# om-ai-lab/OmChat

Measured on AMD Instinct MI355X. Metric: images/sec prefill + decode tokens/sec, OmChat-13B TP=1/8; p50 TTFT, higher is better.
Workload: dtype bf16

## Files before the change

omchat_amd/csrc/attention.hip:

```cpp
#include "kernels.h"

#include "attn_common.h"

namespace {

__device__ __forceinline__ float max3(float a, float b, float c) {
  float r;
  asm("v_max3_f32 %0, %1, %2, %3" : "=v"(r) : "v"(a), "v"(b), "v"(c));
  return r;
}
__device__ __forceinline__ float max2(float a, float b) {
  float r;
  asm("v_max_f32 %0, %1, %2" : "=v"(r) : "v"(a), "v"(b));
  return r;
}
__device__ __forceinline__ float max_xor32_raw(float v) {
  const auto r = __builtin_amdgcn_permlane32_swap(__float_as_uint(v), __float_as_uint(v), false, false);
  return max2(__uint_as_float(r[0]), __uint_as_float(r[1]));
}
__device__ __forceinline__ float max_xor16_raw(float v) {
  const auto r = __builtin_amdgcn_permlane16_swap(__float_as_uint(v), __float_as_uint(v), false, false);
  return max2(__uint_as_float(r[0]), __uint_as_float(r[1]));
}

// ... 228 lines not shown
  extern __shared__ __attribute__((aligned(256))) char smem_all[];

  const int tid = threadIdx.x % NT, lane = tid & 63;
  const int wave_all = __builtin_amdgcn_readfirstlane((int)threadIdx.x >> 6);
  const int kg = KG == 1 ? 0 : wave_all / (NW / KG);
  const int wave = KG == 1 ? wave_all : wave_all % (NW / KG);
  char* const smem = smem_all + kg * 2 * BUF;
  const int qc = lane & 31, hh = lane >> 5;

  const int n_rep = p.q_heads / p.kv_heads;
  const int nb = GQA ? p.nsplit : 1;
  const int per_rank = GQA ? p.kv_heads * nb : 1;
  const int xs = GQA ? p.tpw : 0;
  const int nqb = GQA ? (int)gridDim.x / per_rank - xs : (p.tpw == -1 ? (p.nsplit & 0xffff) : (int)gridDim.x);
  int h_lo = 0, h_hi = GQA ? n_rep : 1, bx, rest;
  if (GQA && (int)blockIdx.x < 2 * xs * per_rank) {
    const int pair = (int)blockIdx.x >> 1;
    bx = pair / per_rank; rest = pair % per_rank;
    if (blockIdx.x & 1) h_lo = (n_rep + 1) / 2; else h_hi = (n_rep + 1) / 2;
  } else if (GQA) {
    const int j = (int)blockIdx.x - 2 * xs * per_rank;
    bx = xs + j / per_rank; rest = j % per_rank;
  } else {
    bx = (int)blockIdx.x; rest = 0;
  }
  int mha_head = (int)blockIdx.y, mha_b = (int)blockIdx.z;
  if (!GQA && p.tpw == -1) {
    const int nq = p.nsplit & 0xffff, nbat = p.nsplit >> 16, grp = (int)blockIdx.x / (8 * nq), r = (int)blockIdx.x % (8 * nq);
    const int pair = grp * 8 + (r & 7);
    bx = r >> 3;
    if (pair >= p.q_heads * nbat) return;
    mha_head = pair % p.q_heads; mha_b = pair / p.q_heads;
  }
  const int qb = p.causal ? nqb - 1 - bx : bx;
  const int b = GQA ? rest / p.kv_heads : mha_b;
  constexpr int QW = GQA ? 32 : (NW / KG) * 32;
  const int kvh = GQA ? rest % p.kv_heads : mha_head / n_rep;
  const int hq = GQA ? kvh * n_rep + wave : mha_head;
  const int q0b = qb * QW;
  const int q0 = q0b + (GQA ? 0 : wave * 32);
  const int kv_len = p.kv_len ? p.kv_len[b] : p.Skv;
  const int kv_start = p.kv_start ? p.kv_start[b] : 0;
  const bool peel = !GQA && KG == 1 && D == 128 && p.peel_last && !p.causal && kv_start == 0 && kv_len > KV_TILE && (kv_len & (KV_TILE - 1)) == 1;
  int kmax = peel ? kv_len - 1 : kv_len;
  if (p.causal) { const int lim = q0b + QW + p.q_pos0; kmax = lim < kmax ? lim : kmax; }
  const int t_end = (kmax + KV_TILE - 1) / KV_TILE;
  const int t_begin = kv_start / KV_TILE;

  const T* Kg = (const T*)p.K + b * p.k_sb + kvh * p.k_sh;
  const T* Vg = (const T*)p.V + b * p.v_sb + kvh * p.v_sh;
  const bool wave_active = (GQA ? (wave >= h_lo && wave < h_hi) : true) && q0 < p.Sq;

  frag_t qf[KS];
  const int qrow = q0 + qc;
  {
    const int rr = qrow < p.Sq ? qrow : p.Sq - 1;
    const T* qp = (const T*)p.Q + b * p.q_sb + (wave_active ? hq : 0) * p.q_sh + (int64_t)rr * p.q_sr;
#pragma unroll
    for (int s = 0; s < KS; ++s) qf[s] = ld8<T>(qp + s * 16 + hh * 8);
  }
  [[maybe_unused]] float qn_ss = 0.f;
  [[maybe_unused]] frag_t qn_wv[(!GQA && D == 128) ? KS : 1];
  if constexpr (!GQA && D == 128) {
    if (p.qn_sumsq) {
      const int rr = qrow < p.Sq ? qrow : p.Sq - 1;
      qn_ss = p.qn_sumsq[((size_t)b * p.Sq + rr) * p.qn_stride];
      const T* wq = (const T*)p.qn_w + (size_t)hq * D;
#pragma unroll
      for (int s = 0; s < KS; ++s) qn_wv[s] = ld8<T>(wq + s * 16 + hh * 8);
// ... 1178 lines not shown
int g_attn_v2 = 1;
void attn_set_v2(int v) { g_attn_v2 = v; }

namespace {
template <typename T>
__global__ __launch_bounds__(128) void attn_uniform_rows_kernel(AttnP p) {
  const int h = blockIdx.x, b = blockIdx.y, d = threadIdx.x;
  const int start = p.kv_start[b];
  if (start <= 0) return;
  const int kvh = h / (p.q_heads / p.kv_heads);
  const T* V = (const T*)p.V + b * p.v_sb + kvh * p.v_sh + d;
  const float w = rnd<T>(1.0f / (float)p.Skv);
  float acc = 0.f;
  for (int j = 0; j < p.Skv; ++j) acc += w * tof(V[(int64_t)j * p.v_sr]);
  const T o = fromf<T>(acc);
  T* O = (T*)p.O + b * p.o_sb + h * p.o_sh + d;
  for (int i = 0; i < start && i < p.Sq; ++i) O[(int64_t)i * p.o_sr] = o;
}
}

int launch_attn_uniform_rows(int dtype, const AttnArgs& a, hipStream_t s) {
  OM_CHECK(a.kv_start && (a.head_dim == 0 || a.head_dim == 128), "uniform rows: left-padded batch (kv_start), head dim 128");
  AttnP p{a.Q, a.K, a.V, a.O, a.q_sb, a.q_sh, a.q_sr, a.k_sb, a.k_sh, a.k_sr, a.v_sb, a.v_sh, a.v_sr, a.o_sb, a.o_sh, a.o_sr,
          a.kv_len, a.kv_start, a.q_heads, a.kv_heads, a.Sq, a.Skv, a.causal, a.q_pos0, 0, a.scale * 1.4426950408889634f, nullptr,
          nullptr, nullptr, nullptr, nullptr, 0, nullptr, nullptr, 0, nullptr, nullptr, 0, 0, 0, nullptr, 0};
  const dim3 grid(a.q_heads, a.batch);
  if (dtype == OMCHAT_F16) hipLaunchKernelGGL(attn_uniform_rows_kernel<f16>, grid, dim3(128), 0, s, p);
  else if (dtype == OMCHAT_BF16) hipLaunchKernelGGL(attn_uniform_rows_kernel<bf16>, grid, dim3(128), 0, s, p);
  else { omchat_set_error("launch_attn_uniform_rows: bad dtype"); return 1; }
  OM_LAUNCH_CHECK();
  return 0;
}

int launch_attn_prefill(int dtype, const AttnArgs& a, hipStream_t s) {
  OM_CHECK(a.q_heads % a.kv_heads == 0, "q_heads must be a multiple of kv_heads");
  OM_CHECK(a.Sq > 0 && a.Skv > 0 && a.batch > 0, "empty attention");
  OM_CHECK(a.q_sr % 8 == 0 && a.k_sr % 8 == 0 && a.v_sr % 8 == 0 && a.o_sr % 4 == 0, "row strides must keep 16-B alignment");
  AttnP p{a.Q, a.K, a.V, a.O, a.q_sb, a.q_sh, a.q_sr, a.k_sb, a.k_sh, a.k_sr, a.v_sb, a.v_sh, a.v_sr, a.o_sb, a.o_sh, a.o_sr,
          a.kv_len, a.kv_start, a.q_heads, a.kv_heads, a.Sq, a.Skv, a.causal, a.q_pos0, 0, a.scale * 1.4426950408889634f, nullptr,
          nullptr, nullptr, nullptr, nullptr, 0, nullptr, nullptr, 0, nullptr, nullptr, 0, 0, 0, nullptr, 0};
  dim3 grid(cdiv(a.Sq, 128), a.q_heads, a.batch);
  p.peel_last = g_attn_peel;
  const int hd = a.head_dim ? a.head_dim : 128;
  OM_CHECK(hd == 128 || hd == 64, "head_dim must be 128 or 64");
  if (a.qn_sumsq) {
    OM_CHECK(a.q_heads == a.kv_heads && hd == 128 && g_attn_v2 && !a.causal && a.qn_w && a.qn_stride >= 1 && a.qn_dim > 0,
             "q norm on load: MHA at head dim 128 on the second-generation kernel");
    p.qn_sumsq = a.qn_sumsq; p.qn_stride = a.qn_stride; p.qn_dim = a.qn_dim; p.qn_w = a.qn_w; p.qn_eps = a.qn_eps; p.qn_scale = a.qn_scale;
  }
  dim3 grid_x = grid;
  if (g_attn_mha_xcd && !a.causal && grid.x < 65536 && a.batch < 32768) { p.tpw = -1; p.nsplit = (int)grid.x | (a.batch << 16); grid_x = dim3(cdiv(a.q_heads * a.batch, 8) * 8 * grid.x, 1, 1); }
  constexpr int LDS128 = 2 * 2 * KV_TILE * 256;
  auto use_kg2 = [&](int per_cu1, int per_cu2) {
    if (!OMCHAT_EXPERIMENTS || g_attn_kg != 2) return false;
    if (a.causal || a.kv_start || a.q_heads != a.kv_heads) return false;
    if (g_attn_kg) return g_attn_kg == 2;
    const long wgs = (long)grid.x * a.q_heads * a.batch, G = device_cus();
    const long r1 = (wgs + G * per_cu1 - 1) / (G * per_cu1), r2 = (wgs + G * per_cu2 - 1) / (G * per_cu2);
    return 2 * r1 > r2 + (r1 > 4 ? 1 : 0) && cdiv(a.Skv, KV_TILE) >= 4;
  };
  if (hd == 64 && g_attn_v2 && a.q_heads == a.kv_heads) {
    const bool kg2 = use_kg2(4, 2); (void)kg2;
    constexpr int LDS64 = 2 * 2 * KV_TILE * 128;
#if OMCHAT_EXPERIMENTS
    if (kg2 && dtype == OMCHAT_F16) OM_LAUNCH_ATTN2((attn2_kernel<f16, 8, false, 64, 2>), grid_x, 512, 2 * LDS64);
    else if (kg2 && dtype == OMCHAT_BF16) OM_LAUNCH_ATTN2((attn2_kernel<bf16, 8, false, 64, 2>), grid_x, 512, 2 * LDS64);
    else
#endif
    if (dtype == OMCHAT_F16) OM_LAUNCH_ATTN2((attn2_kernel<f16, 4, false, 64>), grid_x, 256, LDS64);
    else if (dtype == OMCHAT_BF16) OM_LAUNCH_ATTN2((attn2_kernel<bf16, 4, false, 64>), grid_x, 256, LDS64);
    else { omchat_set_error("launch_attn_prefill: bad dtype"); return 1; }
    OM_LAUNCH_CHECK();
    return 0;
  }
  if (hd == 64) {
    if (dtype == OMCHAT_F16) hipLaunchKernelGGL((attn_kernel<f16, 4, 2, 64>), grid, dim3(256), 0, s, p);
    else if (dtype == OMCHAT_BF16) hipLaunchKernelGGL((attn_kernel<bf16, 4, 2, 64>), grid, dim3(256), 0, s, p);
    else { omchat_set_error("launch_attn_prefill: bad dtype"); return 1; }
    OM_LAUNCH_CHECK();
    return 0;
  }
  const int n_rep = a.q_heads / a.kv_heads;
  if (g_attn_v2 && n_rep == 1) {
    const bool kg2 = use_kg2(2, 1); (void)kg2;
#if OMCHAT_EXPERIMENTS
    if (kg2 && dtype == OMCHAT_F16) OM_LAUNCH_ATTN2((attn2_kernel<f16, 8, false, 128, 2>), grid_x, 512, 2 * LDS128);
    else if (kg2 && dtype == OMCHAT_BF16) OM_LAUNCH_ATTN2((attn2_kernel<bf16, 8, false, 128, 2>), grid_x, 512, 2 * LDS128);
    else
#endif
    if (dtype == OMCHAT_F16) OM_LAUNCH_ATTN2((attn2_kernel<f16, 4, false>), grid_x, 256, LDS128);
    else if (dtype == OMCHAT_BF16) OM_LAUNCH_ATTN2((attn2_kernel<bf16, 4, false>), grid_x, 256, LDS128);
    else { omchat_set_error("launch_attn_prefill: bad dtype"); return 1; }
    OM_LAUNCH_CHECK();
    return 0;
  }
  if (g_attn_v2 && n_rep <= 8) {
    const int nqb_ = cdiv(a.Sq, 32), per_rank = a.kv_heads * a.batch;
    int xs = 0;
    if (a.causal && n_rep >= 4 && !a.kv_start && (long)nqb_ * per_rank <= device_cus() && nqb_ >= 16)
      xs = g_attn_hsplit >= 0 ? std::min(g_attn_hsplit, nqb_ / 2) : nqb_ / 4;
    if (g_attn_hsplit > 0 && a.causal && n_rep >= 4 && !a.kv_start && nqb_ >= 16) xs = std::min(g_attn_hsplit, nqb_ / 2);
    const dim3 g2((nqb_ + xs) * per_rank, 1, 1);
    p.nsplit = a.batch; p.tpw = xs;
#define OM_A2(NW_)                                                                                                       \
  do {                                                                                                                   \
    if (dtype == OMCHAT_F16) OM_LAUNCH_ATTN2((attn2_kernel<f16, NW_, true>), g2, NW_ * 64, LDS128);                      \
    else if (dtype == OMCHAT_BF16) OM_LAUNCH_ATTN2((attn2_kernel<bf16, NW_, true>), g2, NW_ * 64, LDS128);               \
    else { omchat_set_error("launch_attn_prefill: bad dtype"); return 1; }                                               \
  } while (0)
    switch (n_rep) { case 2: OM_A2(2); break; case 3: OM_A2(3); break; case 4: OM_A2(4); break; case 5: OM_A2(5); break;
                     case 6: OM_A2(6); break; case 7: OM_A2(7); break; default: OM_A2(8); break; }
#undef OM_A2
    OM_LAUNCH_CHECK();
    return 0;
  }
  if (dtype == OMCHAT_F16) hipLaunchKernelGGL((attn_kernel<f16, 4, 2, 128>), grid, dim3(256), 0, s, p);
  else if (dtype == OMCHAT_BF16) hipLaunchKernelGGL((attn_kernel<bf16, 4, 2, 128>), grid, dim3(256), 0, s, p);
  else { omchat_set_error("launch_attn_prefill: bad dtype"); return 1; }
  OM_LAUNCH_CHECK();
  return 0;
}

size_t attn_decode_ws_bytes(int batch, int q_heads, int max_len) {
  return (size_t)batch * q_heads * cdiv(max_len, KV_TILE) * WS_STRIDE * sizeof(float);
}

static void kv8_plan(int batch, int kv_heads, int L, bool masked, int* tpw, int* nw) {
  *tpw = 1; *nw = 1;
  if (masked) return;
  const long waves1 = (long)cdiv(L, KV_TILE) * kv_heads * batch;
  if (g_attn_kv8_tpw > 0) { *tpw = g_attn_kv8_tpw & 7; *nw = (g_attn_kv8_tpw & 8) ? 4 : 1; }
  else {
    *tpw = waves1 >= 2L * device_cus() ? 3 : 1;
    const int n4 = cdiv(L, 12 * KV_TILE);
    if (*tpw == 3 && n4 <= 64 && (long)n4 * kv_heads * batch >= device_cus() / 2) *nw = 4;
  }
// ... 369 lines not shown
```

omchat_amd/csrc/attn_common.h:

```cpp
#pragma once
#include "kernels.h"

namespace {


struct AttnP {
  const void* Q; const void* K; const void* V; void* O;
  int64_t q_sb, q_sh, q_sr, k_sb, k_sh, k_sr, v_sb, v_sh, v_sr, o_sb, o_sh, o_sr;
  const int* kv_len;
  const int* kv_start;
  int q_heads, kv_heads, Sq, Skv, causal, q_pos0, nsplit;
  float c;
  float* ws;
  const float* rope;
  const int* pos;
  const void* k_new; const void* v_new; int64_t new_sb;
  void* k_cache_w; void* v_cache_w;
  int rope_max;
  const float* k_scale; const float* v_scale; int64_t scale_sb, scale_sh;
  int tpw;
  const unsigned char* key_mask; int64_t mask_sb;
  const float* qn_sumsq = nullptr; int qn_stride = 0, qn_dim = 0; const void* qn_w = nullptr; float qn_eps = 0.f, qn_scale = 1.f;
  int peel_last = 0;
#if OMCHAT_EXPERIMENTS
  unsigned long long* dbg;
#endif
};

template <typename T> __device__ __forceinline__ typename V8<T>::type widen8(u32x2 w);
template <> __device__ __forceinline__ bf16x8 widen8<bf16>(u32x2 w) {
  typedef bf16 v2 __attribute__((ext_vector_type(2)));
  const v2 a = __builtin_amdgcn_cvt_scalef32_pk_bf16_fp8(w.x, 1.0f, false), b = __builtin_amdgcn_cvt_scalef32_pk_bf16_fp8(w.x, 1.0f, true);
  const v2 c = __builtin_amdgcn_cvt_scalef32_pk_bf16_fp8(w.y, 1.0f, false), d = __builtin_amdgcn_cvt_scalef32_pk_bf16_fp8(w.y, 1.0f, true);
  return (bf16x8){a[0], a[1], b[0], b[1], c[0], c[1], d[0], d[1]};
}
template <> __device__ __forceinline__ f16x8 widen8<f16>(u32x2 w) {
  typedef f16 v2 __attribute__((ext_vector_type(2)));
  const v2 a = __builtin_amdgcn_cvt_scalef32_pk_f16_fp8(w.x, 1.0f, false), b = __builtin_amdgcn_cvt_scalef32_pk_f16_fp8(w.x, 1.0f, true);
  const v2 c = __builtin_amdgcn_cvt_scalef32_pk_f16_fp8(w.y, 1.0f, false), d = __builtin_amdgcn_cvt_scalef32_pk_f16_fp8(w.y, 1.0f, true);
  return (f16x8){a[0], a[1], b[0], b[1], c[0], c[1], d[0], d[1]};
}

template <typename T>
__device__ __forceinline__ typename V8<T>::type rope_chunk(typename V8<T>::type x, typename V8<T>::type o, const float* cs, bool second_half) {
#pragma clang fp contract(off)
  typename V8<T>::type r;
  const float sgn = second_half ? 1.f : -1.f;
#pragma unroll
  for (int j = 0; j < 8; ++j) {
    const float co = rnd<T>(cs[2 * j]), si = rnd<T>(cs[2 * j + 1]);
    r[j] = fromf<T>(rnd<T>(tof(x[j]) * co) + rnd<T>(sgn * tof(o[j]) * si));
  }
  return r;
}

constexpr int KV_TILE = 64;
// ... 227 lines not shown
```

omchat_amd/csrc/capi.hip:

```cpp
#include "kernels.h"
#include <stdlib.h>
#include "../../include/omchat_hip.h"
#include <math.h>
#include <vector>

#define S(x) ((hipStream_t)(x))
#if OMCHAT_EXPERIMENTS
int g_launch_any_order = 0;
#endif

extern "C" int omchat_op_gemm(int dtype, const void* A, int lda, const void* W, int ldw, void* C, int ldc, int M, int N, int K,
                              const void* bias, const void* ls, const void* resid, int ldr, int epi, int force_tile, void* stream) {
  GemmArgs g{A, lda, W, ldw, C, ldc, M, N, K, bias, ls, resid, ldr, epi, force_tile, nullptr, 0, -1};
  return launch_gemm(dtype, g, S(stream));
}

extern "C" int omchat_op_gemm_fused(int dtype, const void* A, int lda, const void* W, int ldw, void* C, int ldc, int M, int N, int K,
                                    const void* bias, const void* ls, const void* resid, int ldr, int epi, int force_tile, const float* row_scale,
                                    const float* rs_stats, int rs_ld, int rs_nslots, int rs_dim, float rs_eps,
                                    float* stats, int stats_ld, int* nslots, void* stream) {
  GemmArgs g{A, lda, W, ldw, C, ldc, M, N, K, bias, ls, resid, ldr, epi, force_tile, nullptr, 0, -1};
  g.row_scale = row_scale; g.stats = stats; g.stats_ld = stats_ld; g.stats_nslots = nslots;
  g.rs_stats = rs_stats; g.rs_ld = rs_ld; g.rs_nslots = rs_nslots; g.rs_dim = rs_dim; g.rs_eps = rs_eps;
  return launch_gemm(dtype, g, S(stream));
// ... 39 lines not shown
  if (key == 6) { model_set_pack_replica(value); return 0; }
  if (key == 8) { attn_set_v2(value); return 0; }
  if (key == 9) { model_set_fuse_peer_norm(value); return 0; }
  if (key == 10) { attn_set_tpw(value); return 0; }
  if (key == 11) { gemv_set_no_xs(value); return 0; }
  if (key == 12) { attn_set_klds(value); return 0; }
  if (key == 25) { attn_set_dma(value); return 0; }
  if (key == 26) { attn_set_dma_slots(value); return 0; }
  if (key == 27) { attn_set_dma_rot(value); return 0; }
  if (key == 28) { gemv_set_skew(value); return 0; }
  if (key == 29) { model_set_tp_f32(value); return 0; }
  if (key == 30) { attn_set_hsplit(value); return 0; }
  if (key == 33) { attn_set_mha_xcd(value); return 0; }
  if (key == 16) { gemv_set_norm_loop(value); return 0; }
  if (key == 17) { gemv_set_rows_balance(value); return 0; }
  if (key == 19) { attn_set_merge_mid_min(value); return 0; }
  if (key == 21) { attn_set_merge_dg(value); return 0; }
  if (key == 13) { gemm_set_persist(value); return 0; }
  if (key == 14) { model_set_norm_in_gemv(value); return 0; }
  if (key == 22) { model_set_fuse_attn_oproj(value); return 0; }
  if (key == 23) { model_set_decode_layer(value); return 0; }
  if (key == 24) { gemv_set_dyn(value); return 0; }
  if (key == 34) { gemv_set_shard_shapes(value); return 0; }
  if (key == 35) { model_set_shard_as_tp1(value); return 0; }
  if (key == 36) { attn_set_kg(value); return 0; }
  if (key == 37) { gemm_set_wide_store(value); return 0; }
  if (key == 43) { gemm_set_skip_dead(value); return 0; }
  if (key == 44) { model_set_vit_fused(value); return 0; }
  if (key == 45) { model_set_tp_sp(value); return 0; }
  if (key == 46) { attn_set_peel(value); return 0; }
  if (key == 47) { attn_set_kv8_tpw(value); return 0; }
  if (key == 48) { attn_set_kv8_fuse(value); return 0; }
  if (key == 49) { model_set_extend_attn(value); return 0; }
  if (key == 38) { gemv_set_gu_rr(value); return 0; }
  if (key == 39) { gemv_set_longk_direct(value); return 0; }
  if (key == 40) { norm_set_wave(value); return 0; }
#if OMCHAT_EXPERIMENTS
  if (key == 41) { g_launch_any_order = value; return 0; }
  if (key == 42) { model_set_ao_oproj(value); return 0; }
#endif
  omchat_set_error("omchat_op_set_tuning: unknown key");
  return 1;
}

extern "C" int omchat_allreduce_noop(void*, void*, size_t, int, void*) { return 0; }

extern "C" int omchat_gemm_tune_load(const char* path) { OM_CHECK(path, "null path"); return gemm_tune_load(path); }
extern "C" int omchat_gemm_tune_dump(const char* path) { OM_CHECK(path, "null path"); return gemm_tune_dump(path); }
extern "C" long omchat_gemm_tune_runs(void) { return gemm_tune_runs(); }

extern "C" size_t omchat_op_gemm_sk_ws(void) { return gemm_sk_ws_bytes(); }

extern "C" int omchat_op_gemm_sk(int dtype, const void* A, int lda, const void* W, int ldw, void* C, int ldc, int M, int N, int K,
                                 const void* bias, const void* ls, const void* resid, int ldr, int epi, int force_tile, void* ws,
                                 size_t ws_bytes, int stream_k, void* stream) {
  GemmArgs g{A, lda, W, ldw, C, ldc, M, N, K, bias, ls, resid, ldr, epi, force_tile, ws, ws_bytes, stream_k};
  return launch_gemm(dtype, g, S(stream));
}

extern "C" int omchat_op_gemv(int dtype, const void* X, int ldx, const void* W, int ldw, void* Y, int ldy, int b, int N, int K,
                              const void* bias, const void* resid, int ldr, int epi, int out_f32, void* stream) {
  GemvArgs g{X, ldx, W, ldw, Y, ldy, b, N, K, bias, resid, ldr, epi, out_f32};
  return launch_gemv(dtype, g, S(stream));
}

extern "C" int omchat_op_gemv_norm(int dtype, const void* X, const void* W, int ldw, void* Y, int N, int K, const void* norm_w, float eps,
// ... 383 lines not shown
```

omchat_amd/csrc/kernels.h:

```cpp
#pragma once
#ifndef OMCHAT_EXPERIMENTS
#define OMCHAT_EXPERIMENTS 0
#endif
#include "common.h"
#if OMCHAT_EXPERIMENTS
#include <hip/hip_ext.h>
extern int g_launch_any_order;
#undef hipLaunchKernelGGL
#define hipLaunchKernelGGL(kernelName, numBlocks, numThreads, memPerBlock, streamId, ...)                                                      \
  do {                                                                                                                                         \
    if (g_launch_any_order)                                                                                                                    \
      hipExtLaunchKernelGGL((kernelName), dim3(numBlocks), dim3(numThreads), (memPerBlock), (streamId), nullptr, nullptr, hipExtAnyOrderLaunch, \
                            __VA_ARGS__);                                                                                                      \
    else                                                                                                                                       \
      hipLaunchKernelGGLInternal((kernelName), numBlocks, numThreads, memPerBlock, streamId, __VA_ARGS__);                                     \
  } while (0)
#endif

enum {
  EPI_NONE = 0,
  EPI_GELU = 1,
  EPI_LS_RESID = 2,
  EPI_RESID = 3,
  EPI_SWIGLU = 4,
// ... 66 lines not shown
void model_set_pack_replica(int v);
void model_set_norm_in_gemv(int v);
void model_set_vit_fused(int v);
void model_set_tp_sp(int v);
int launch_fold_cols(int dtype, const void* W, const void* n, void* out, int rows, int cols, hipStream_t s);

int launch_layernorm(int dtype, const void* x, int ldx, const void* w, const void* b, void* y, int ldy, int rows, int H, float eps, hipStream_t stream);
int launch_rmsnorm(int dtype, const void* x, int ldx, const void* w, void* y, int ldy, int rows, int H, float eps, hipStream_t s, int pack_nb = 0);
int launch_rmsnorm_q8(int dtype, const void* x, int ldx, const void* w, void* y8, int ldy, float* scale, int rows, int H, float eps, hipStream_t s);
int launch_quant_rows_q8(int dtype, const void* x, int ldx, void* y8, int ldy, float* scale, int rows, int H, hipStream_t s);
int launch_resid_rmsnorm(int dtype, void* x, int ldx, const float* part, int ks, const void* w, void* xn, int ldn, int rows, int H, float eps,
                         hipStream_t s, int pack_nb = 0);
int launch_resid16_norm(int dtype, void* x, int ldx, const void* y, int ldy, const void* w, const void* b, void* xn, int ldn, int rows, int H, float eps,
                        hipStream_t s);
int launch_vit_qknorm(int dtype, void* qkv, int ld, const void* wq, const void* wk, int rows, int C, int C_total,
                      float eps, float q_scale, const float* sumsq_in, hipStream_t s, int only_k = 0);
int launch_vit_qk_sumsq(int dtype, const void* qkv, int ld, int rows, int C, float* sumsq_out, hipStream_t s);
int launch_vit_knorm_slots(int dtype, void* k, int ld, const void* wk, int rows, int C, int C_total, float eps, const float* stats, int stats_ld, int nslots,
                           float* sumsq_q, hipStream_t s);
struct AttnArgs {
  const void* Q; int64_t q_sb, q_sh, q_sr;
  const void* K; int64_t k_sb, k_sh, k_sr;
  const void* V; int64_t v_sb, v_sh, v_sr;
  void* O; int64_t o_sb, o_sh, o_sr;
  int batch, q_heads, kv_heads;
  int Sq, Skv;
  const int* kv_len;
  const int* kv_start;
  int causal;
  int q_pos0;
  float scale;
  int head_dim;
  const float* qn_sumsq = nullptr; int qn_stride = 0, qn_dim = 0; const void* qn_w = nullptr; float qn_eps = 0.f, qn_scale = 1.f;
};
int launch_attn_prefill(int dtype, const AttnArgs& a, hipStream_t s);
int launch_attn_uniform_rows(int dtype, const AttnArgs& a, hipStream_t s);
void attn_set_v2(int v);
void model_set_fuse_peer_norm(int v);
void attn_set_tpw(int v);
void attn_set_klds(int v);
void attn_set_dma(int v);
void attn_set_dma_slots(int v);
void attn_set_dma_rot(int v);
void attn_set_hsplit(int v);
void attn_set_mha_xcd(int v);
void attn_set_kg(int v);
void attn_set_peel(int v);
void attn_set_kv8_tpw(int v);
void attn_set_kv8_fuse(int v);
void model_set_extend_attn(int v);
bool attn_decode_kv8_fuses_rope(int batch, int kv_heads, int L, bool masked);
void attn_set_merge_mid_min(int v);
void attn_set_merge_dg(int v);
void gemv_set_norm_loop(int v);
void gemv_set_dyn(int v);
void gemv_set_skew(int v);
void gemv_set_rows_balance(int v);
void gemv_set_no_xs(int v);
void gemv_set_shard_shapes(int v);
void gemv_set_gu_rr(int v);
void gemv_set_longk_direct(int v);
void norm_set_wave(int v);
void model_set_ao_oproj(int v);
int gemv_get_shard_shapes();

struct AttnDecodeArgs {
  const void* Q; int64_t q_sb, q_sh;
  const void* K; int64_t k_sb, k_sh, k_sr;
  const void* V; int64_t v_sb, v_sh, v_sr;
  void* O; int64_t o_sb, o_sh;
  int batch, q_heads, kv_heads;
  int L;
  const int* kv_len;
  float scale;
  float* ws; size_t ws_bytes;
  const float* rope; int rope_max;
  const int* pos;
  const void* k_new; const void* v_new; int64_t new_sb;
  int o_pack_nb;
  const float* k_scale; const float* v_scale; int64_t scale_sb, scale_sh;
  void* k16_w = nullptr; void* v16_w = nullptr;
  const unsigned char* key_mask; int64_t mask_sb;
  unsigned* done_flags = nullptr; unsigned done_epoch = 0; int done_mode = 0;
// ... 135 lines not shown
```

omchat_amd/csrc/model.hip:

```cpp
#include "kernels.h"
#include "../../include/omchat_hip.h"
#include <rccl/rccl.h>
#include <limits.h>
#include <math.h>
#include <string.h>
#include <algorithm>
#include <functional>
#include <string>
#include <unordered_map>
#include <vector>

static thread_local std::string g_err;
void omchat_set_error(const std::string& s) { g_err = s; }
extern "C" const char* omchat_last_error(void) { return g_err.c_str(); }
extern "C" const char* omchat_version(void) { return "omchat_hip 0.1 (gfx950)"; }

namespace {

__global__ void cast_from_f32_f16(const float* s, f16* d, int64_t n) {
  for (int64_t i = (int64_t)blockIdx.x * blockDim.x + threadIdx.x; i < n; i += (int64_t)gridDim.x * blockDim.x) d[i] = (f16)s[i];
}
__global__ void cast_from_f32_bf16(const float* s, bf16* d, int64_t n) {
  for (int64_t i = (int64_t)blockIdx.x * blockDim.x + threadIdx.x; i < n; i += (int64_t)gridDim.x * blockDim.x) d[i] = (bf16)s[i];
}
// ... 90 lines not shown
  struct DecLayerP { void *wqkv = nullptr, *wo = nullptr, *wgu = nullptr, *wd = nullptr; };
  std::vector<DecLayerP> dlp;
  void* t_lmP = nullptr;
  bool pk_ready = false, pk_unavailable = false;
  void* t_lm8 = nullptr; float* t_lm8_s = nullptr;
  bool fp8_decode = false, fp8_stale = false;
  void *k8cache = nullptr, *v8cache = nullptr;
  float *ks8 = nullptr, *vs8 = nullptr;
  bool fp8_kv = false, kv8_valid = false, fp8_prefill = false;
  void* tw_q8 = nullptr; float* tw_q8s = nullptr;
  int64_t scale_layer_stride() const { return (int64_t)c.max_batch * c.t_kv_heads * c.max_seq; }
  struct DecodeGraph { hipGraph_t graph = nullptr; hipGraphExec_t exec = nullptr; int cap_len = 0; };
  std::unordered_map<int, DecodeGraph> graphs;
  bool graph_on = false;
  hipStream_t graph_stream = nullptr;
  hipEvent_t graph_ev_in = nullptr, graph_ev_out = nullptr;
  int32_t *d_tok_in = nullptr, *d_tok_out = nullptr;
  long graph_steps = 0, graph_replays = 0, graph_captures = 0;
  void *v_cls = nullptr, *v_pos = nullptr, *v_wpatch = nullptr, *v_bpatch = nullptr;
  std::vector<VitLayer> vl;
  void *p_w0 = nullptr, *p_b0 = nullptr, *p_w2 = nullptr, *p_b2 = nullptr;
  void *t_embed = nullptr, *t_norm = nullptr, *t_lm = nullptr;
  std::vector<DecLayer> dl;
  float* rope = nullptr;

  void *vw_cols = nullptr, *vw_pe = nullptr, *vw_x = nullptr, *vw_x2 = nullptr, *vw_xn = nullptr, *vw_qkv = nullptr, *vw_ao = nullptr,
       *vw_h = nullptr, *vw_feat = nullptr, *vw_proj = nullptr;
  float* vw_sumsq = nullptr;
  float *vw_stats_x = nullptr, *vw_stats_qk = nullptr, *vw_rstd = nullptr;
  int vw_stats_x_ld = 0, vw_stats_qk_ld = 0, vw_stats_x_ld_used = 1;
  struct VitFold { void *wqkv = nullptr, *w1 = nullptr; };
  std::vector<VitFold> vfold;
  bool vfold_stale = true;
  void *tw_x = nullptr, *tw_x2 = nullptr, *tw_xn = nullptr, *tw_qkv = nullptr, *tw_ao = nullptr, *tw_act = nullptr, *tw_last = nullptr;
  float* tw_logits = nullptr;
  void* sk_ws = nullptr; size_t sk_ws_bytes = 0;
  float* tp_table = nullptr;
  float* tp_f32_ws = nullptr; size_t tp_f32_bytes = 0;
  void* arg_scratch = nullptr;
  float* tw_part = nullptr;
  float* tw_attn_ws = nullptr;
  size_t tw_attn_ws_bytes = 0;
  void* fd_ws = nullptr;
  unsigned* fd_err = nullptr;
  unsigned fd_epoch = 0;
  long n_fused_launches = 0;
  void* dl_ws = nullptr;
  long n_layer_launches = 0;
  unsigned long long* dbg_stamps = nullptr;
  unsigned* dyn_ctr = nullptr;
  int *d_pos = nullptr, *d_len = nullptr, *d_idx = nullptr, *d_start = nullptr;
  int* d_verify_n = nullptr;
  struct Sampling { bool on = false; uint64_t seed = 0; float temperature = 1.f; int top_k = 0; double top_p = 1.0; float penalty = 1.f; };
  Sampling smp;
  void* smp_ws = nullptr;
  uint32_t* smp_bm = nullptr; int smp_bmw = 0;
  int *smp_last = nullptr, *smp_step = nullptr;
  struct Beam { bool on = false; int b = 0, N = 0, KB = 0, max_new = 0, P = 0, es = 0, ns = 1, t = 0; float lp = 1.f; std::vector<int> eos; };
  Beam beam;
  struct Grown { void* p = nullptr; size_t cap = 0; };
  Grown bm_state, bm_table, bm_dn, bm_parents, bm_stash;
  Grown ext_ws;
  bool bm_stash8 = false;
  std::vector<int> bm_hpos, bm_hlen;
  int grow(Grown& g, size_t n) {
    if (n <= g.cap) return 0;
    if (g.p) { hipFree(g.p); bytes -= g.cap; g.p = nullptr; g.cap = 0; }
// ... 217 lines not shown
    }
    TRY(ctx->alloc((void**)&ctx->rope, tab.size() * 4));
    OM_HIP(hipMemcpy(ctx->rope, tab.data(), tab.size() * 4, hipMemcpyHostToDevice));
  }

  if (c.v_layers > 0) {
    const size_t Bm = (size_t)c.max_tiles, M = Bm * ctx->v_ntok;
    TRY(ctx->alloc(&ctx->vw_cols, Bm * ctx->v_np * ctx->v_kpad * 2));
    TRY(ctx->alloc(&ctx->vw_pe, Bm * ctx->v_np * C * 2));
    const size_t SL = 64;
    TRY(ctx->alloc(&ctx->vw_x, (M + SL) * C * 2));
    TRY(ctx->alloc(&ctx->vw_x2, (M + SL) * C * 2));
    TRY(ctx->alloc(&ctx->vw_xn, (M + SL) * C * 2));
    TRY(ctx->alloc(&ctx->vw_qkv, M * 3 * ctx->v_Cq * 2));
    TRY(ctx->alloc(&ctx->vw_ao, M * ctx->v_Cq * 2));
    TRY(ctx->alloc(&ctx->vw_h, M * I * 2));
    TRY(ctx->alloc(&ctx->vw_feat, M * C * 2));
    TRY(ctx->alloc(&ctx->vw_proj, M * c.t_hidden * 2));
    TRY(ctx->alloc((void**)&ctx->vw_sumsq, M * 2 * 4 + 64));
    ctx->vw_stats_x_ld = ctx->vw_stats_qk_ld = (int)((M + 63) / 64 * 64);
    TRY(ctx->alloc((void**)&ctx->vw_stats_x, (size_t)(cdiv(C, 48) + 2) * ctx->vw_stats_x_ld * 4));
    TRY(ctx->alloc((void**)&ctx->vw_stats_qk, (size_t)(cdiv(3 * ctx->v_Cq, 64) + 1) * ctx->vw_stats_qk_ld * 4));
    TRY(ctx->alloc((void**)&ctx->vw_rstd, M * 4 + 64));
  }
  if (c.t_layers > 0) {
    const size_t R = std::max<size_t>(32, (size_t)(c.max_prefill_rows > c.max_batch ? c.max_prefill_rows : c.max_batch));
    TRY(ctx->alloc(&ctx->tw_x, (R + 64) * H * 2));
    TRY(ctx->alloc(&ctx->tw_x2, (R + 64) * H * 2));
    TRY(ctx->alloc(&ctx->tw_xn, (R + 64) * H * 2));
    TRY(ctx->alloc(&ctx->tw_qkv, R * ctx->t_qkvdim * 2));
    TRY(ctx->alloc(&ctx->tw_ao, R * ctx->t_qdim * 2));
    TRY(ctx->alloc(&ctx->tw_act, R * It * 2));
    TRY(ctx->alloc(&ctx->tw_last, (size_t)c.max_batch * H * 2));
    const size_t DR = std::max(c.max_batch, VERIFY_MAX_T);
    TRY(ctx->alloc((void**)&ctx->tw_logits, DR * c.t_vocab * 4));
    ctx->tw_attn_ws_bytes = attn_decode_ws_bytes((int)DR, c.t_heads, c.max_seq);
    TRY(ctx->alloc((void**)&ctx->tw_attn_ws, ctx->tw_attn_ws_bytes));
    TRY(ctx->alloc((void**)&ctx->tw_part, (size_t)DEC_KS_MAX * DR * H * 4));
    if (OMCHAT_EXPERIMENTS) {
      const size_t fb = fused_decode_ws_bytes(c.t_heads);
      TRY(ctx->alloc(&ctx->fd_ws, fb));
      TRY(ctx->alloc((void**)&ctx->fd_err, 64));
      OM_HIP(hipMemset(ctx->fd_ws, 0, fb));
      OM_HIP(hipMemset(ctx->fd_err, 0, 64));
      const size_t lb = decode_layer_ws_bytes(c.t_heads, H, ctx->t_qdim, ctx->t_kvdim, It);
      TRY(ctx->alloc(&ctx->dl_ws, lb));
      OM_HIP(hipMemset(ctx->dl_ws, 0, lb));
      TRY(ctx->alloc((void**)&ctx->dyn_ctr, (size_t)c.t_layers * 65 * 64 * 4));
      OM_HIP(hipMemset(ctx->dyn_ctr, 0, (size_t)c.t_layers * 65 * 64 * 4));
      TRY(ctx->alloc((void**)&ctx->dbg_stamps, (size_t)c.t_layers * 256));
      OM_HIP(hipMemset(ctx->dbg_stamps, 0, (size_t)c.t_layers * 256));
    }
    TRY(ctx->alloc(&ctx->arg_scratch, argmax_scratch_bytes((int)DR)));
    TRY(ctx->alloc((void**)&ctx->tp_table, (size_t)ctx->tp_size * DR * 2 * 4));
    TRY(ctx->alloc((void**)&ctx->d_verify_n, 16));
    TRY(ctx->alloc((void**)&ctx->d_pos, (size_t)c.max_batch * 4));
    TRY(ctx->alloc((void**)&ctx->d_len, (size_t)c.max_batch * 4));
    TRY(ctx->alloc((void**)&ctx->d_idx, (size_t)c.max_batch * 4));
    TRY(ctx->alloc((void**)&ctx->d_start, (size_t)c.max_batch * 4));
    const size_t cache = (size_t)c.t_layers * ctx->cache_layer_stride() * 2;
    TRY(ctx->alloc(&ctx->kcache, cache));
    TRY(ctx->alloc(&ctx->vcache, cache));
    OM_HIP(hipMemset(ctx->kcache, 0, cache));
    OM_HIP(hipMemset(ctx->vcache, 0, cache));
    ctx->h_len.assign(c.max_batch, 0);
  }
// ... 684 lines not shown
  SampleArgs a;
  a.logits = lg; a.ld = c.t_vocab; a.b = b; a.V = c.t_vocab; a.V_total = c.t_vocab_total;
  a.rank = ctx->tp_rank; a.tp = ctx->tp_size;
  a.seed = ctx->smp.seed; a.temperature = ctx->smp.temperature; a.top_k = ctx->smp.top_k; a.top_p = ctx->smp.top_p; a.penalty = ctx->smp.penalty;
  if (ctx->smp.penalty != 1.f) { a.bitmap = ctx->smp_bm; a.bm_words = ctx->smp_bmw; }
  a.last_set = ctx->smp_last; a.step = ctx->smp_step;
  if (advance) { a.adv_pos = ctx->d_pos; a.adv_len = ctx->d_len; }
  a.out = next_tokens; a.ws = ctx->smp_ws; a.table = ctx->tp_table;
  a.xchg = smp_xchg; a.xchg_user = ctx;
  return launch_sample(a, s);
}

extern "C" int omchat_greedy(omchat_ctx* ctx, const float* logits, int b, int32_t* next_tokens, void* stream) {
  OM_CHECK(ctx && logits && next_tokens && b >= 1 && b <= ctx->c.max_batch, "bad argument");
  return greedy_pick(ctx, logits, b, next_tokens, (hipStream_t)stream);
}

extern "C" int omchat_lm_head(omchat_ctx* ctx, const void* hidden, int n, float* logits, void* stream) {
  OM_CHECK(ctx && hidden && logits, "null argument");
  return lm_head_rows(ctx, hidden, n, logits, (hipStream_t)stream);
}

int g_extend_attn = -1;
void model_set_extend_attn(int v) { g_extend_attn = v; }
static bool extend_attn_split(int S, int keep, int kv_heads) {
  if (keep <= 0 || kv_heads <= 0) return false;
  if (g_extend_attn >= 0) return g_extend_attn != 0;
  const long wgs = (long)cdiv(S, 32) * kv_heads;
  if (4 * wgs <= device_cus()) return true;
  return 2 * wgs <= device_cus() && keep + S >= 16384;
}
extern "C" int omchat_extend_attn_form(int S_new, int keep, int Hkv) { return extend_attn_split(S_new, keep, Hkv) ? 1 : 0; }

static int prefill_impl(omchat_ctx* ctx, const void* embeds, int b, int S, const int32_t* lengths, float* logits_last, void* hidden_out,
                        void* stream, bool left, int keep = 0) {
  OM_CHECK(ctx && embeds && lengths, "null argument");
  const omchat_config& c = ctx->c;
  OM_CHECK(c.t_layers > 0, "context has no decoder");
  OM_CHECK(b >= 1 && b <= c.max_batch, "batch exceeds max_batch");
  OM_CHECK(S >= 1 && keep + S <= c.max_seq, "sequence exceeds max_seq");
  OM_CHECK((int64_t)b * S <= c.max_prefill_rows, "b * S exceeds max_prefill_rows");
  OM_CHECK(omchat_weights_missing(ctx) == 0, std::string(omchat_last_error()));
  for (int i = 0; i < b; ++i) OM_CHECK(lengths[i] >= 1 && lengths[i] <= S, "lengths must be in [1, S]");
  hipStream_t s = (hipStream_t)stream;
  if (ctx->fp8_prefill && ctx->fp8_stale) TRY(ensure_fp8_weights(ctx));
  const int H = c.t_hidden, It = c.t_mlp, rows = b * S, qkvd = ctx->t_qkvdim, qd = ctx->t_qdim;
  const bool lead = ctx->tp_rank == 0;

  const bool split_attn = extend_attn_split(S, keep, c.t_kv_heads) && c.t_heads / c.t_kv_heads <= 8;
  if (split_attn) TRY(ctx->grow(ctx->ext_ws, attn_extend_ws_bytes(S, c.t_heads, c.t_kv_heads, keep)));
  std::vector<int> pos(b), len1(b), klen(b), kstart(b);
  for (int i = 0; i < b; ++i) {
    ctx->h_len[i] = left ? 0 : keep + lengths[i];
    pos[i] = keep + lengths[i]; len1[i] = keep + lengths[i] + 1;
    klen[i] = left ? S : keep + lengths[i]; kstart[i] = left ? S - lengths[i] : 0;
  }
  ctx->left_padded = left;
  ctx->pre_S = keep + S; ctx->pre_b = b; ctx->masked_steps = 0; ctx->dec_mode = 0; ctx->mask_on_device = false;
  OM_HIP(hipMemcpyAsync(ctx->d_len, klen.data(), (size_t)b * 4, hipMemcpyHostToDevice, s));
  if (left) OM_HIP(hipMemcpyAsync(ctx->d_start, kstart.data(), (size_t)b * 4, hipMemcpyHostToDevice, s));

  void* x = ctx->tw_x;
  void* y = ctx->tw_x2;
  OM_HIP(hipMemcpyAsync(x, embeds, (size_t)rows * H * 2, hipMemcpyDeviceToDevice, s));
  const bool sp = g_tp_sp && ctx->tp_size > 1 && !g_tp_f32 && !(ctx->fp8_prefill && !ctx->dl8.empty() && !ctx->fp8_stale);
  for (int i = 0; i < c.t_layers; ++i) {
    auto& L = ctx->dl[i];
    char* kc = (char*)ctx->kcache + (size_t)i * ctx->cache_layer_stride() * 2;
    char* vc = (char*)ctx->vcache + (size_t)i * ctx->cache_layer_stride() * 2;
    const bool f8p = ctx->fp8_prefill && !ctx->dl8.empty() && !ctx->fp8_stale;
    auto gemm_f8 = [&](const void* W8, const float* sw, void* Cb, int ldc, int N, const void* bias, int epi) -> int {
      GemmArgs g{ctx->tw_q8, H, W8, H, Cb, ldc, rows, N, H, bias, nullptr, nullptr, 0, epi, 0, nullptr, 0, -1, 1, ctx->tw_q8s, sw};
      return launch_gemm(ctx->dt, g, s);
    };
    if (f8p) {
      TRY(launch_rmsnorm_q8(ctx->dt, x, H, L.ln1, ctx->tw_q8, H, ctx->tw_q8s, rows, H, c.t_eps, s));
      TRY(gemm_f8(ctx->dl8[i].wqkv, ctx->dl8[i].sqkv, ctx->tw_qkv, qkvd, qkvd, L.bqkv, EPI_NONE));
    } else {
      if (!sp || i == 0) TRY(launch_rmsnorm(ctx->dt, x, H, L.ln1, ctx->tw_xn, H, rows, H, c.t_eps, s));
      if (sp) TRY(gemm_after_sp(ctx, ctx->tw_xn, H, L.wqkv, H, ctx->tw_qkv, qkvd, rows, qkvd, H, L.bqkv, EPI_NONE, s));
      else TRY(gemm(ctx, ctx->tw_xn, H, L.wqkv, H, ctx->tw_qkv, qkvd, rows, qkvd, H, L.bqkv, nullptr, nullptr, 0, EPI_NONE, s));
    }
    RopeArgs r{ctx->tw_qkv, qkvd, rows, S, c.t_heads, c.t_kv_heads, nullptr, keep, ctx->rope, c.max_seq, kc, vc, ctx->cache_sb(), ctx->cache_sh()};
    TRY(launch_rope_kv(ctx->dt, r, s));
    if (split_attn) {
      AttnExtendArgs e{};
      e.Q = ctx->tw_qkv; e.q_sb = qkvd; e.q_sh = 128;
      e.K = kc; e.k_sh = ctx->cache_sh(); e.k_sr = 128;
      e.V = vc; e.v_sh = e.k_sh; e.v_sr = 128;
      e.O = ctx->tw_ao; e.o_sb = qd; e.o_sh = 128;
      e.Sq = S; e.q_heads = c.t_heads; e.kv_heads = c.t_kv_heads; e.L = keep; e.scale = 0.08838834764831845f;
      e.ws = (float*)ctx->ext_ws.p; e.ws_bytes = ctx->ext_ws.cap;
      TRY(launch_attn_extend(ctx->dt, e, s));
    }
    AttnArgs a{};
    a.Q = ctx->tw_qkv; a.q_sb = (int64_t)S * qkvd; a.q_sh = 128; a.q_sr = qkvd;
    a.K = kc; a.k_sb = ctx->cache_sb(); a.k_sh = ctx->cache_sh(); a.k_sr = 128;
    a.V = vc; a.v_sb = a.k_sb; a.v_sh = a.k_sh; a.v_sr = 128;
    a.O = ctx->tw_ao; a.o_sb = (int64_t)S * qd; a.o_sh = 128; a.o_sr = qd;
    a.batch = b; a.q_heads = c.t_heads; a.kv_heads = c.t_kv_heads; a.Sq = S; a.Skv = keep + S; a.kv_len = ctx->d_len; a.causal = 1; a.q_pos0 = keep;
    a.kv_start = left ? ctx->d_start : nullptr;
    a.scale = 0.08838834764831845f;
    if (!split_attn) TRY(launch_attn_prefill(ctx->dt, a, s));
    if (left && ctx->tp_size == 1) TRY(launch_attn_uniform_rows(ctx->dt, a, s));
    if (ctx->tp_size == 1) {
      TRY(gemm(ctx, ctx->tw_ao, qd, L.wo, qd, x, H, rows, H, qd, nullptr, nullptr, x, H, EPI_RESID, s));
    } else if (sp) {
      TRY(gemm_sp(ctx, ctx->tw_ao, qd, L.wo, qd, y, x, H, rows, qd, nullptr, nullptr, EPI_RESID, L.ln2, nullptr, ctx->tw_xn, c.t_eps, s));
    } else {
      TRY(gemm_allreduce(ctx, ctx->tw_ao, qd, L.wo, qd, y, H, rows, qd, nullptr, nullptr, x, EPI_RESID, s));
      std::swap(x, y);
    }
    if (f8p) TRY(launch_rmsnorm_q8(ctx->dt, x, H, L.ln2, ctx->tw_q8, H, ctx->tw_q8s, rows, H, c.t_eps, s));
    else if (!sp) TRY(launch_rmsnorm(ctx->dt, x, H, L.ln2, ctx->tw_xn, H, rows, H, c.t_eps, s));
    ctx->prof_mark(OMCHAT_PROF_PREFILL_GATEUP, s);
    if (f8p) TRY(gemm_f8(ctx->dl8[i].wgu, ctx->dl8[i].sgu, ctx->tw_act, It, 2 * It, nullptr, EPI_SWIGLU));
    else if (sp) TRY(gemm_after_sp(ctx, ctx->tw_xn, H, L.wgu, H, ctx->tw_act, It, rows, 2 * It, H, nullptr, EPI_SWIGLU, s));
    else TRY(gemm(ctx, ctx->tw_xn, H, L.wgu, H, ctx->tw_act, It, rows, 2 * It, H, nullptr, nullptr, nullptr, 0, EPI_SWIGLU, s));
    ctx->prof_mark(OMCHAT_PROF_PREFILL_GATEUP, s);
    if (ctx->tp_size == 1) {
      TRY(gemm(ctx, ctx->tw_act, It, L.wd, It, x, H, rows, H, It, nullptr, nullptr, x, H, EPI_RESID, s));
    } else if (sp) {
      const bool more = i + 1 < c.t_layers;
      TRY(gemm_sp(ctx, ctx->tw_act, It, L.wd, It, y, x, H, rows, It, nullptr, nullptr, EPI_RESID, more ? ctx->dl[i + 1].ln1 : nullptr, nullptr, ctx->tw_xn, c.t_eps, s));
      if (!more) TRY(sp_gather_x(ctx, x, H, rows, s));
    } else {
      TRY(gemm_allreduce(ctx, ctx->tw_act, It, L.wd, It, y, H, rows, It, nullptr, nullptr, x, EPI_RESID, s));
      std::swap(x, y);
    }
  }
  TRY(sp_drain(ctx, s));
  if (hidden_out) TRY(launch_rmsnorm(ctx->dt, x, H, ctx->t_norm, hidden_out, H, rows, H, c.t_eps, s));
  if (logits_last) {
    hipLaunchKernelGGL(last_row_index_kernel, dim3(1), dim3(64 > b ? 64 : b), 0, s, ctx->d_len, S, b, ctx->d_idx, keep);
    TRY(launch_gather_rows(ctx->dt, ctx->d_idx, x, nullptr, ctx->tw_last, b, H, s));
    TRY(launch_rmsnorm(ctx->dt, ctx->tw_last, H, ctx->t_norm, ctx->tw_last, H, b, H, c.t_eps, s));
    TRY(lm_head_rows(ctx, ctx->tw_last, b, logits_last, s));
  }
  ctx->kv8_valid = false;
  ctx->beam.on = false;
  if (ctx->fp8_kv) {
    for (int i = 0; i < c.t_layers; ++i) {
      const size_t off = (size_t)i * ctx->cache_layer_stride(), so = (size_t)i * ctx->scale_layer_stride();
      TRY(launch_kv_quant(ctx->dt, (char*)ctx->kcache + off * 2, (char*)ctx->vcache + off * 2, (char*)ctx->k8cache + off, (char*)ctx->v8cache + off,
                          ctx->ks8 + so, ctx->vs8 + so, b, c.t_kv_heads, ctx->cache_sb(), ctx->cache_sh(), (int64_t)c.t_kv_heads * c.max_seq, c.max_seq,
                          nullptr, 0, nullptr, S, s));
    }
    ctx->kv8_valid = true;
  }
  OM_HIP(hipMemcpyAsync(ctx->d_pos, pos.data(), (size_t)b * 4, hipMemcpyHostToDevice, s));
  OM_HIP(hipMemcpyAsync(ctx->d_len, len1.data(), (size_t)b * 4, hipMemcpyHostToDevice, s));
  OM_HIP(hipStreamSynchronize(s));
  return 0;
}

extern "C" int omchat_prefill(omchat_ctx* ctx, const void* embeds, int b, int S, const int32_t* lengths, float* logits_last, void* hidden_out,
                              void* stream) {
  return prefill_impl(ctx, embeds, b, S, lengths, logits_last, hidden_out, stream, false);
}

extern "C" int omchat_prefill_left(omchat_ctx* ctx, const void* embeds, int b, int S, const int32_t* lengths, float* logits_last,
                                   void* hidden_out, void* stream) {
  return prefill_impl(ctx, embeds, b, S, lengths, logits_last, hidden_out, stream, true);
}

extern "C" int omchat_prefill_extend(omchat_ctx* ctx, const void* embeds, int S_new, int keep, float* logits_last, void* hidden_out, void* stream) {
  OM_CHECK(ctx, "null argument");
  OM_CHECK(S_new >= 1, "prefill_extend: S_new < 1");
// ... 847 lines not shown
```

Baseline: 341.7.

## Compute only last-token rows in the final prefill layer

When only last-token logits are needed (TP=1, no hidden output, no cached prefix), the final layer runs attention only for the query block containing each sequence's last token. It then gathers that row and runs the output projection, MLP and residual for just b rows instead of all S rows. The cost targeted is the full-sequence attention, o-proj and MLP GEMMs in the last layer, which are wasted because only the last row feeds the LM head. It adds a last_block mode to the GQA kernel grid and extra gather launches, and the K/V cache for the last layer is still written.

New measurement: 342.1 (median of 3 runs). Within noise of the previous version (+0.1%).

```diff
diff --git a/omchat_amd/csrc/attention.hip b/omchat_amd/csrc/attention.hip
--- a/omchat_amd/csrc/attention.hip
+++ b/omchat_amd/csrc/attention.hip
@@ -284,9 +284,13 @@
     if (pair >= p.q_heads * nbat) return;
     mha_head = pair % p.q_heads; mha_b = pair / p.q_heads;
   }
-  const int qb = p.causal ? nqb - 1 - bx : bx;
   const int b = GQA ? rest / p.kv_heads : mha_b;
   constexpr int QW = GQA ? 32 : (NW / KG) * 32;
+  int qb = p.causal ? nqb - 1 - bx : bx;
+  if (GQA && p.last_block) {
+    const int last = (p.kv_len ? p.kv_len[b] : p.Skv) - p.q_pos0 - 1;
+    qb = (last < 0 ? 0 : (last < p.Sq ? last : p.Sq - 1)) / QW;
+  }
   const int kvh = GQA ? rest % p.kv_heads : mha_head / n_rep;
   const int hq = GQA ? kvh * n_rep + wave : mha_head;
   const int q0b = qb * QW;
@@ -1531,8 +1535,16 @@
   return 0;
 }
 
+bool attn_prefill_last_block_ok(int q_heads, int kv_heads, int head_dim) {
+  if (!g_attn_v2 || kv_heads <= 0 || q_heads % kv_heads || (head_dim && head_dim != 128)) return false;
+  const int n_rep = q_heads / kv_heads;
+  return n_rep >= 2 && n_rep <= 8;
+}
+
 int launch_attn_prefill(int dtype, const AttnArgs& a, hipStream_t s) {
   OM_CHECK(a.q_heads % a.kv_heads == 0, "q_heads must be a multiple of kv_heads");
+  OM_CHECK(!a.last_block || (a.causal && a.kv_len && attn_prefill_last_block_ok(a.q_heads, a.kv_heads, a.head_dim)),
+           "last_block: causal GQA launch with per-sequence key counts (attn_prefill_last_block_ok)");
   OM_CHECK(a.Sq > 0 && a.Skv > 0 && a.batch > 0, "empty attention");
   OM_CHECK(a.q_sr % 8 == 0 && a.k_sr % 8 == 0 && a.v_sr % 8 == 0 && a.o_sr % 4 == 0, "row strides must keep 16-B alignment");
   AttnP p{a.Q, a.K, a.V, a.O, a.q_sb, a.q_sh, a.q_sr, a.k_sb, a.k_sh, a.k_sr, a.v_sb, a.v_sh, a.v_sr, a.o_sb, a.o_sh, a.o_sr,
@@ -1599,8 +1611,9 @@
     if (a.causal && n_rep >= 4 && !a.kv_start && (long)nqb_ * per_rank <= device_cus() && nqb_ >= 16)
       xs = g_attn_hsplit >= 0 ? std::min(g_attn_hsplit, nqb_ / 2) : nqb_ / 4;
     if (g_attn_hsplit > 0 && a.causal && n_rep >= 4 && !a.kv_start && nqb_ >= 16) xs = std::min(g_attn_hsplit, nqb_ / 2);
-    const dim3 g2((nqb_ + xs) * per_rank, 1, 1);
-    p.nsplit = a.batch; p.tpw = xs;
+    if (a.last_block) xs = 0;
+    const dim3 g2(a.last_block ? per_rank : (nqb_ + xs) * per_rank, 1, 1);
+    p.nsplit = a.batch; p.tpw = xs; p.last_block = a.last_block;
 #define OM_A2(NW_)                                                                                                       \
   do {                                                                                                                   \
     if (dtype == OMCHAT_F16) OM_LAUNCH_ATTN2((attn2_kernel<f16, NW_, true>), g2, NW_ * 64, LDS128);                      \
diff --git a/omchat_amd/csrc/attn_common.h b/omchat_amd/csrc/attn_common.h
--- a/omchat_amd/csrc/attn_common.h
+++ b/omchat_amd/csrc/attn_common.h
@@ -22,6 +22,7 @@
   const unsigned char* key_mask; int64_t mask_sb;
   const float* qn_sumsq = nullptr; int qn_stride = 0, qn_dim = 0; const void* qn_w = nullptr; float qn_eps = 0.f, qn_scale = 1.f;
   int peel_last = 0;
+  int last_block = 0;
 #if OMCHAT_EXPERIMENTS
   unsigned long long* dbg;
 #endif
diff --git a/omchat_amd/csrc/capi.hip b/omchat_amd/csrc/capi.hip
--- a/omchat_amd/csrc/capi.hip
+++ b/omchat_amd/csrc/capi.hip
@@ -95,6 +95,7 @@
   if (key == 47) { attn_set_kv8_tpw(value); return 0; }
   if (key == 48) { attn_set_kv8_fuse(value); return 0; }
   if (key == 49) { model_set_extend_attn(value); return 0; }
+  if (key == 50) { model_set_prefill_tail(value); return 0; }
   if (key == 38) { gemv_set_gu_rr(value); return 0; }
   if (key == 39) { gemv_set_longk_direct(value); return 0; }
   if (key == 40) { norm_set_wave(value); return 0; }
diff --git a/omchat_amd/csrc/kernels.h b/omchat_amd/csrc/kernels.h
--- a/omchat_amd/csrc/kernels.h
+++ b/omchat_amd/csrc/kernels.h
@@ -122,8 +122,10 @@
   float scale;
   int head_dim;
   const float* qn_sumsq = nullptr; int qn_stride = 0, qn_dim = 0; const void* qn_w = nullptr; float qn_eps = 0.f, qn_scale = 1.f;
+  int last_block = 0;
 };
 int launch_attn_prefill(int dtype, const AttnArgs& a, hipStream_t s);
+bool attn_prefill_last_block_ok(int q_heads, int kv_heads, int head_dim);
 int launch_attn_uniform_rows(int dtype, const AttnArgs& a, hipStream_t s);
 void attn_set_v2(int v);
 void model_set_fuse_peer_norm(int v);
@@ -139,6 +141,7 @@
 void attn_set_kv8_tpw(int v);
 void attn_set_kv8_fuse(int v);
 void model_set_extend_attn(int v);
+void model_set_prefill_tail(int v);
 bool attn_decode_kv8_fuses_rope(int batch, int kv_heads, int L, bool masked);
 void attn_set_merge_mid_min(int v);
 void attn_set_merge_dg(int v);
diff --git a/omchat_amd/csrc/model.hip b/omchat_amd/csrc/model.hip
--- a/omchat_amd/csrc/model.hip
+++ b/omchat_amd/csrc/model.hip
@@ -146,7 +146,7 @@
   struct VitFold { void *wqkv = nullptr, *w1 = nullptr; };
   std::vector<VitFold> vfold;
   bool vfold_stale = true;
-  void *tw_x = nullptr, *tw_x2 = nullptr, *tw_xn = nullptr, *tw_qkv = nullptr, *tw_ao = nullptr, *tw_act = nullptr, *tw_last = nullptr;
+  void *tw_x = nullptr, *tw_x2 = nullptr, *tw_xn = nullptr, *tw_qkv = nullptr, *tw_ao = nullptr, *tw_act = nullptr, *tw_last = nullptr, *tw_last_ao = nullptr;
   float* tw_logits = nullptr;
   void* sk_ws = nullptr; size_t sk_ws_bytes = 0;
   float* tp_table = nullptr;
@@ -430,6 +430,7 @@
     TRY(ctx->alloc(&ctx->tw_ao, R * ctx->t_qdim * 2));
     TRY(ctx->alloc(&ctx->tw_act, R * It * 2));
     TRY(ctx->alloc(&ctx->tw_last, (size_t)c.max_batch * H * 2));
+    TRY(ctx->alloc(&ctx->tw_last_ao, (size_t)c.max_batch * ctx->t_qdim * 2));
     const size_t DR = std::max(c.max_batch, VERIFY_MAX_T);
     TRY(ctx->alloc((void**)&ctx->tw_logits, DR * c.t_vocab * 4));
     ctx->tw_attn_ws_bytes = attn_decode_ws_bytes((int)DR, c.t_heads, c.max_seq);
@@ -1180,6 +1181,9 @@
 }
 extern "C" int omchat_extend_attn_form(int S_new, int keep, int Hkv) { return extend_attn_split(S_new, keep, Hkv) ? 1 : 0; }
 
+int g_prefill_tail = 1;
+void model_set_prefill_tail(int v) { g_prefill_tail = v; }
+
 static int prefill_impl(omchat_ctx* ctx, const void* embeds, int b, int S, const int32_t* lengths, float* logits_last, void* hidden_out,
                         void* stream, bool left, int keep = 0) {
   OM_CHECK(ctx && embeds && lengths, "null argument");
@@ -1196,6 +1200,7 @@
   const bool lead = ctx->tp_rank == 0;
 
   const bool split_attn = extend_attn_split(S, keep, c.t_kv_heads) && c.t_heads / c.t_kv_heads <= 8;
+  const bool tail = g_prefill_tail && logits_last && !hidden_out && ctx->tp_size == 1 && keep == 0;
   if (split_attn) TRY(ctx->grow(ctx->ext_ws, attn_extend_ws_bytes(S, c.t_heads, c.t_kv_heads, keep)));
   std::vector<int> pos(b), len1(b), klen(b), kstart(b);
   for (int i = 0; i < b; ++i) {
@@ -1217,13 +1222,13 @@
     char* kc = (char*)ctx->kcache + (size_t)i * ctx->cache_layer_stride() * 2;
     char* vc = (char*)ctx->vcache + (size_t)i * ctx->cache_layer_stride() * 2;
     const bool f8p = ctx->fp8_prefill && !ctx->dl8.empty() && !ctx->fp8_stale;
-    auto gemm_f8 = [&](const void* W8, const float* sw, void* Cb, int ldc, int N, const void* bias, int epi) -> int {
-      GemmArgs g{ctx->tw_q8, H, W8, H, Cb, ldc, rows, N, H, bias, nullptr, nullptr, 0, epi, 0, nullptr, 0, -1, 1, ctx->tw_q8s, sw};
+    auto gemm_f8 = [&](const void* W8, const float* sw, void* Cb, int ldc, int M, int N, const void* bias, int epi) -> int {
+      GemmArgs g{ctx->tw_q8, H, W8, H, Cb, ldc, M, N, H, bias, nullptr, nullptr, 0, epi, 0, nullptr, 0, -1, 1, ctx->tw_q8s, sw};
       return launch_gemm(ctx->dt, g, s);
     };
     if (f8p) {
       TRY(launch_rmsnorm_q8(ctx->dt, x, H, L.ln1, ctx->tw_q8, H, ctx->tw_q8s, rows, H, c.t_eps, s));
-      TRY(gemm_f8(ctx->dl8[i].wqkv, ctx->dl8[i].sqkv, ctx->tw_qkv, qkvd, qkvd, L.bqkv, EPI_NONE));
+      TRY(gemm_f8(ctx->dl8[i].wqkv, ctx->dl8[i].sqkv, ctx->tw_qkv, qkvd, rows, qkvd, L.bqkv, EPI_NONE));
     } else {
       if (!sp || i == 0) TRY(launch_rmsnorm(ctx->dt, x, H, L.ln1, ctx->tw_xn, H, rows, H, c.t_eps, s));
       if (sp) TRY(gemm_after_sp(ctx, ctx->tw_xn, H, L.wqkv, H, ctx->tw_qkv, qkvd, rows, qkvd, H, L.bqkv, EPI_NONE, s));
@@ -1249,6 +1254,24 @@
     a.batch = b; a.q_heads = c.t_heads; a.kv_heads = c.t_kv_heads; a.Sq = S; a.Skv = keep + S; a.kv_len = ctx->d_len; a.causal = 1; a.q_pos0 = keep;
     a.kv_start = left ? ctx->d_start : nullptr;
     a.scale = 0.08838834764831845f;
+    if (tail && i == c.t_layers - 1) {
+      a.last_block = attn_prefill_last_block_ok(c.t_heads, c.t_kv_heads, 0) ? 1 : 0;
+      TRY(launch_attn_prefill(ctx->dt, a, s));
+      hipLaunchKernelGGL(last_row_index_kernel, dim3(1), dim3(64 > b ? 64 : b), 0, s, ctx->d_len, S, b, ctx->d_idx, keep);
+      void* xl = ctx->tw_last;
+      TRY(launch_gather_rows(ctx->dt, ctx->d_idx, ctx->tw_ao, nullptr, ctx->tw_last_ao, b, qd, s));
+      TRY(launch_gather_rows(ctx->dt, ctx->d_idx, x, nullptr, xl, b, H, s));
+      TRY(gemm(ctx, ctx->tw_last_ao, qd, L.wo, qd, xl, H, b, H, qd, nullptr, nullptr, xl, H, EPI_RESID, s));
+      if (f8p) {
+        TRY(launch_rmsnorm_q8(ctx->dt, xl, H, L.ln2, ctx->tw_q8, H, ctx->tw_q8s, b, H, c.t_eps, s));
+        TRY(gemm_f8(ctx->dl8[i].wgu, ctx->dl8[i].sgu, ctx->tw_act, It, b, 2 * It, nullptr, EPI_SWIGLU));
+      } else {
+        TRY(launch_rmsnorm(ctx->dt, xl, H, L.ln2, ctx->tw_xn, H, b, H, c.t_eps, s));
+        TRY(gemm(ctx, ctx->tw_xn, H, L.wgu, H, ctx->tw_act, It, b, 2 * It, H, nullptr, nullptr, nullptr, 0, EPI_SWIGLU, s));
+      }
+      TRY(gemm(ctx, ctx->tw_act, It, L.wd, It, xl, H, b, H, It, nullptr, nullptr, xl, H, EPI_RESID, s));
+      break;
+    }
     if (!split_attn) TRY(launch_attn_prefill(ctx->dt, a, s));
     if (left && ctx->tp_size == 1) TRY(launch_attn_uniform_rows(ctx->dt, a, s));
     if (ctx->tp_size == 1) {
@@ -1262,7 +1285,7 @@
     if (f8p) TRY(launch_rmsnorm_q8(ctx->dt, x, H, L.ln2, ctx->tw_q8, H, ctx->tw_q8s, rows, H, c.t_eps, s));
     else if (!sp) TRY(launch_rmsnorm(ctx->dt, x, H, L.ln2, ctx->tw_xn, H, rows, H, c.t_eps, s));
     ctx->prof_mark(OMCHAT_PROF_PREFILL_GATEUP, s);
-    if (f8p) TRY(gemm_f8(ctx->dl8[i].wgu, ctx->dl8[i].sgu, ctx->tw_act, It, 2 * It, nullptr, EPI_SWIGLU));
+    if (f8p) TRY(gemm_f8(ctx->dl8[i].wgu, ctx->dl8[i].sgu, ctx->tw_act, It, rows, 2 * It, nullptr, EPI_SWIGLU));
     else if (sp) TRY(gemm_after_sp(ctx, ctx->tw_xn, H, L.wgu, H, ctx->tw_act, It, rows, 2 * It, H, nullptr, EPI_SWIGLU, s));
     else TRY(gemm(ctx, ctx->tw_xn, H, L.wgu, H, ctx->tw_act, It, rows, 2 * It, H, nullptr, nullptr, nullptr, 0, EPI_SWIGLU, s));
     ctx->prof_mark(OMCHAT_PROF_PREFILL_GATEUP, s);
@@ -1280,8 +1303,10 @@
   TRY(sp_drain(ctx, s));
   if (hidden_out) TRY(launch_rmsnorm(ctx->dt, x, H, ctx->t_norm, hidden_out, H, rows, H, c.t_eps, s));
   if (logits_last) {
-    hipLaunchKernelGGL(last_row_index_kernel, dim3(1), dim3(64 > b ? 64 : b), 0, s, ctx->d_len, S, b, ctx->d_idx, keep);
-    TRY(launch_gather_rows(ctx->dt, ctx->d_idx, x, nullptr, ctx->tw_last, b, H, s));
+    if (!tail) {
+      hipLaunchKernelGGL(last_row_index_kernel, dim3(1), dim3(64 > b ? 64 : b), 0, s, ctx->d_len, S, b, ctx->d_idx, keep);
+      TRY(launch_gather_rows(ctx->dt, ctx->d_idx, x, nullptr, ctx->tw_last, b, H, s));
+    }
     TRY(launch_rmsnorm(ctx->dt, ctx->tw_last, H, ctx->t_norm, ctx->tw_last, H, b, H, c.t_eps, s));
     TRY(lm_head_rows(ctx, ctx->tw_last, b, logits_last, s));
   }
```
